# IIT-PAVIS/Acoustic-Image-Generation

Hardware: AMD Instinct MI355X
Metric: train-step images/sec (higher is better)
Workload: dtype f32

## Files before the change

acoustic-image-generation_amd/acimg/_lib.py:

```python
import ctypes as C
import os

_HERE = os.path.dirname(os.path.abspath(__file__))
LIB_PATH = os.environ.get("ACIMG_LIB") or os.path.join(_HERE, "lib", "libacimg.so")

ACT_NONE, ACT_RELU, ACT_SIGMOID = 0, 1, 2


class ConvDesc(C.Structure):

    _fields_ = [(n, C.c_int32) for n in (
        "N", "H", "W", "C", "ldx", "K", "ldy", "OH", "OW", "R", "S", "stride", "pad_t", "pad_l",
        "ldw", "act")]

    def __repr__(self):
        return "ConvDesc(" + ", ".join("%s=%d" % (n, getattr(self, n)) for n, _ in self._fields_) + ")"


class Config(C.Structure):

    _fields_ = [(n, C.c_int32) for n in (
        "splitk_cut", "splitk_target", "splitk_handoff", "wgrad_minpix", "wgrad_halo", "split3_tile_bm",
        "split3_tile_bn", "tail_split", "tail_s", "trunk_persistent", "trunk_bk", "trunk_stagger", "trunk_dma_pos",
        "trunk_ring", "trunk_ring_bm", "trunk_halo")]
# ... 33 lines not shown
    "acimg_conv2d_split3_weight_bytes": (_SZ, [_DP]),
    "acimg_conv2d_split3_prepare": (_I, [_DP, _P, _P, _P]),
    "acimg_conv2d_bf16_prepare": (_I, [_DP, _P, _P, _P]),
    "acimg_conv2d_fwd_split3_stats_rows": (_I, [_DP]),
    "acimg_conv2d_fwd_split3_tiling": (_I, [_DP, C.POINTER(C.c_int)]),
    "acimg_conv2d_fwd_split3p_stats_rows": (_I, [_DP]),
    "acimg_conv2d_fwd_split3": (_I, [_DP, _P, _P, _P, _P, _P, _P, _I, _P, _P]),
    "acimg_conv2d_fwd_bf16": (_I, [_DP, _P, _P, _P, _P, _P, _P, _I, _P, _P]),
    "acimg_conv2d_split3_dgrad_weight_bytes": (_SZ, [_DP]),
    "acimg_conv2d_split3_prepare_dgrad": (_I, [_DP, _P, _P, _P]),
    "acimg_conv2d_dgrad_split3": (_I, [_DP, _P, _I, _P, _P, _I, _P, _I, _P, _I, _P]),
    "acimg_conv2d_dgrad_bf16": (_I, [_DP, _P, _I, _P, _P, _I, _P, _I, _P, _I, _P]),
    "acimg_conv2d_split3_prepare_multi": (_I, [_I, _P, _P, _P, _P, _P]),
    "acimg_conv2d_fwd_split3p_workspace": (_SZ, [_DP]),
    "acimg_conv2d_fwd_split3p": (_I, [_DP, _P, _SZ, _P, _P, _P, _P, _SZ, _P]),
    "acimg_conv2d_fwd_split1p": (_I, [_DP, _P, _SZ, _P, _P, _P, _P, _SZ, _P]),
    "acimg_conv2d_fwd_split3p_stats": (_I, [_DP, _P, _SZ, _P, _P, _P, _SZ, _P]),
    "acimg_gram_stats_workspace": (_SZ, [_L, _I]),
    "acimg_gram_stats": (_I, [_P, _SZ, _L, _I, _P, _I, _I, _P, _P, _P, _P, _F, _F, _P, _P, _P, _SZ, _P]),
    "acimg_conv2d_fwd_split3p_tail": (_I, [_DP, _P, _SZ, _P, _P, _P, _P, _SZ, _P, _SZ, _P, _SZ, _P]),
    "acimg_conv2d_fwd_split3p_tail_proj": (_I, [_DP, _P, _SZ, _P, _P, _P, _P, _P, _P, _P, _SZ, _P, _SZ, _P]),
    "acimg_split_plane_bytes": (_SZ, [_L, _I]),
    "acimg_bn_relu_split": (_I, [_P, _P, _P, _I, _P, _SZ, _L, _I, _P]),
    "acimg_bn_add_relu_split": (_I, [_P, _P, _P, _P, _P, _P, _P, _SZ, _P, _SZ, _P, _I, _I, _I, _I, _I, _I, _I, _P]),
    "acimg_bn_relu_maxpool_split": (_I, [_P, _P, _P, _P, _SZ, _I, _I, _I, _I, _I, _I, _I, _I, _P]),
    "acimg_conv2d_dgrad": (_I, [_DP, _P, _I, _P, _P, _I, _P, _I, _P, _I, _P, _SZ, _P, _P]),
    "acimg_conv2d_dgrad_workspace": (_SZ, [_DP]),
    "acimg_conv2d_wgrad": (_I, [_DP, _P, _P, _I, _P, _P, _P, _SZ, _P]),
    "acimg_conv2d_wgrad_workspace": (_SZ, [_DP]),
    "acimg_conv2d_wgrad_split3": (_I, [_DP, _P, _P, _I, _P, _P, _P, _SZ, _P]),
# ... 140 lines not shown
```

acoustic-image-generation_amd/acimg/ops.py:

```python
import ctypes as C
import math

import torch

from . import _lib
from ._lib import ACT_NONE, ACT_RELU, ACT_SIGMOID, ConvDesc


def up4(v):
    return (int(v) + 3) & ~3


class Ptr(object):

    __slots__ = ("t", "off")

    def __init__(self, t, off=0):
        self.t = t
        self.off = int(off)

    def addr(self):
        return self.t.data_ptr() + 4 * self.off


# ... 418 lines not shown
    plan.add("conv2d_dgrad_bf16" if bf16 else "conv2d_dgrad_split3", fn, C.byref(d), gy, int(ldgy), wsplit_t, dx,
             int(lddx), residual, int(ldres), mask, int(ldmask))


def conv2d_fwd_split3p_workspace(d):
    return int(_L().acimg_conv2d_fwd_split3p_workspace(C.byref(d)))


def conv2d_fwd_split3p(plan, d, x_planes, x_lo_off, wsplit, y, stats=None, tail_ws=None, terms=3, side=False):
    nbytes = 0 if tail_ws is None else (tail_ws.numel() * tail_ws.element_size() if hasattr(tail_ws, "numel") else 0)
    fn = _L().acimg_conv2d_fwd_split3p if terms == 3 else _L().acimg_conv2d_fwd_split1p
    plan.add("conv2d_fwd_split3p" if terms == 3 else "conv2d_fwd_split1p", fn, C.byref(d), x_planes, int(x_lo_off),
             wsplit, y, stats, tail_ws, int(nbytes), side=side)


def conv2d_fwd_split3p_stats(plan, d, x_planes, x_lo_off, wsplit, stats, tail_ws=None, side=False):
    nbytes = 0 if tail_ws is None else (tail_ws.numel() * tail_ws.element_size() if hasattr(tail_ws, "numel") else 0)
    plan.add("conv2d_fwd_split3p_stats", _L().acimg_conv2d_fwd_split3p_stats, C.byref(d), x_planes, int(x_lo_off), wsplit,
             stats, tail_ws, int(nbytes), side=side)


def gram_stats_workspace(rows, Cn):
    return int(_L().acimg_gram_stats_workspace(int(rows), int(Cn)))


def gram_stats(plan, x_planes, x_lo_off, rows, Cn, w, ldw, K, gamma, beta, moving_mean, moving_var, scale, shift, ws,
               decay=0.997, eps=1e-5, side=False):
    plan.add("gram_stats", _L().acimg_gram_stats, x_planes, int(x_lo_off), int(rows), int(Cn), w, int(ldw), int(K), gamma,
             beta, moving_mean, moving_var, float(decay), float(eps), scale, shift, ws,
             int(ws.numel() * ws.element_size()), side=side)
# ... 321 lines not shown
```

acoustic-image-generation_amd/acimg/unet_acresnet.py:

```python
import os
from collections import OrderedDict

import numpy as np
import torch

from . import ops
from .ops import ACT_NONE, ACT_RELU, ACT_SIGMOID, Ptr
from .params import FusedHeads, Var, up4
from .session import get_default_session
from .vision import load_state_file

Z = 150


class Act(object):

    def __init__(self, t, N, H, W, C, ld=None, off=0):
        self.t, self.N, self.H, self.W, self.C = t, N, H, W, C
        self.ld = up4(C) if ld is None else ld
        self.off = off

    @property
    def ptr(self):
        return Ptr(self.t, self.off)
# ... 3 lines not shown
        return up4(self.C)

    @property
    def pixels(self):
        return self.N * self.H * self.W


class UNetAc(object):

    def __init__(self, input_shape=None, num_frames=12, embedding=False, num_skip=1, precision="split", side_lane=True):
        assert precision in ("split", "f32")
        self.precision = precision
        self.split_min_rows = 16384
        self.side_lane = bool(side_lane)
        self._wsplit_bufs = {}
        self.scope = 'UNetAcRes'
        self.num_frames = num_frames
        self.height = input_shape[0]
        self.width = input_shape[1]
        self.channels = input_shape[2]
        self.embedding = bool(embedding)
        self.num_skip = int(num_skip)
        assert self.num_skip in (0, 1, 2)
        self.session = None

    def _conv_specs(self):
        ns = self.num_skip
        return OrderedDict([
            ("final", (3, 3, 64, 12)),
            ("layer7/conv_2", (3, 3, 64, 64)), ("layer7/conv_1", (3, 3, 128, 64)),
# ... 132 lines not shown
        return ops.conv_desc(x.N, x.H, x.W, x.Cp if x.off == 0 and x.ld == x.Cp else x.C, K, 3, 3, stride, "SAME",
                             ldx=x.ld, ldy=(y.ld if y is not None else up4(K)), ldw=up4(K), act=act)

    def _use_split(self, d):
        return (self.precision == "split" and d.stride == 1 and d.C % 32 == 0 and d.K % 32 == 0 and
                d.N * d.OH * d.OW >= self.split_min_rows)

    def _wsplit(self, name, nbytes, kind):
        key = (name, kind)
        if key not in self._wsplit_bufs:
            self._wsplit_bufs[key] = torch.zeros(int(nbytes), dtype=torch.uint8, device=self.session.device)
        return self._wsplit_bufs[key]

    def _prepare_job(self, plan, d, name, image, mode):
        if getattr(self, "_prep_jobs", None) is None:
            (ops.conv2d_split3_prepare_dgrad if mode else ops.conv2d_split3_prepare)(plan, d, self._P(name + "/kernel"),
                                                                                      image)
            return
        self._prep_jobs.add(d, self._P(name + "/kernel"), image, mode)

    def _conv(self, plan, name, x, y, stride=1, act=ACT_RELU):
        d = self._desc(x, y.C, stride, y, act)
        self._descs[name] = (d, x, y)
        if self._use_split(d):
            ws = self._wsplit(name, ops.conv2d_split3_weight_bytes(d), "fwd")
            self._prepare_job(plan, d, name, ws, 0)
            ops.conv2d_fwd_split3(plan, d, x.ptr, ws, y.ptr, bias=self._P(name + "/bias"))
        else:
            ops.conv2d_fwd(plan, d, x.ptr, self._P(name + "/kernel"), self._P(name + "/bias"), y.ptr)

    def _record_forward(self, plan):
        N = self.N
        self._descs = {}
        h, w = self.pool1.H, self.pool1.W
        self._prep_jobs = None
        if self.precision == "split":
            self._prep_jobs = ops.PrepareJobs()
            ops.conv2d_split3_prepare_multi(plan, self._prep_jobs)
        self._conv(plan, "layer1/conv_1", self.inp, self.c11)
        self._conv(plan, "layer1/conv_2", self.c11, self.conv1)
        self._conv(plan, "layer1/pool_2", self.conv1, self.pool1, stride=3)
        self._conv(plan, "layer2/conv_1", self.pool1, self.c21)
        self._conv(plan, "layer2/conv_2", self.c21, self.conv2_0)
        ops.minmax_fwd(plan, self.conv2_0.ptr, self.conv2_0.ld, self.cat145, 148, self.mm_a, N, h * w, 133)
        ops.minmax_fwd(plan, self.feat.ptr, 12, Ptr(self.cat145, 133), 148, self.mm_b, N, h * w, 12)
        kin = h * w * 148
        self.d_heads = ops.conv_desc(N, 1, 1, kin, self.hn if not self.embedding else Z, 1, 1, 1, "VALID",
                                     ldx=kin, ldy=self.hn, ldw=self.hn)
        ops.conv2d_fwd(plan, self.d_heads, self.cat145, self._P("heads/kernel"), self._P("heads/bias"),
                       self.heads_out)
        if self.embedding:
            ops.minmax_fwd(plan, self.heads_out, self.hn, self.zbuf, 152, self.mm_z, N, 1, Z)
        else:
            ops.latent_fwd(plan, self.heads_out, self.eps, self.zbuf, 152, self.sigma, self.kl, N, Z)
        self.d_dense = ops.conv_desc(N, 1, 1, 152, 2304, 1, 1, 1, "VALID", ldx=152, ldy=2304, ldw=2304,
                                     act=ACT_RELU)
        ops.conv2d_fwd(plan, self.d_dense, self.zbuf, self._P("dense/kernel"), self._P("dense/bias"), self.dns.t)
        self._conv(plan, "conv2d", self.dns, self.net)
        self._conv(plan, "layer4/conv_1", self.l4in, self.c41)
        self._conv(plan, "layer4/conv_2", self.c41, self.conv4)
        self._conv(plan, "layer5/conv_1", self.conv4, self.c51)
        self._conv(plan, "layer5/conv_2", self.c51, self.conv5)
        self.d_up = ops.deconv_desc(N, h, w, 128, 128, 2, 2, 3, ldx=128, ldy=self.up.ld, ldw=128)
        ops.deconv_fwd(plan, self.d_up, self.conv5.ptr, self._P("upsample_1/kernel"), self._P("upsample_1/bias"),
                       self.up.ptr)
        self._conv(plan, "layer6/conv_1", self.l6in, self.c61)
        self._conv(plan, "layer6/conv_2", self.c61, self.conv6)
        self._conv(plan, "layer7/conv_1", self.conv6, self.c71)
        self._conv(plan, "layer7/conv_2", self.c71, self.conv7)
        self._conv(plan, "final", self.conv7, self.yhat, act=ACT_SIGMOID)

    def record_backward(self, plan, g_logit, g_feat, kl_weight, on_ready=None):
        on_ready = on_ready or (lambda name: None)
        N = self.N
        z = self.session.zeros
        H, W, h, w = self.height, self.width, self.pool1.H, self.pool1.W
        ns = self.num_skip

        def gbuf(a, full=False):
            return Act(z(a.N, a.H, a.W, up4(a.C)), a.N, a.H, a.W, a.C)

        def back(name, gy, dx=None, mask=None, res=None):
            d, x, y = self._descs[name]
# ... 86 lines not shown
```

acoustic-image-generation_amd/csrc/common.hpp:

```cpp
#pragma once
#include <hip/hip_runtime.h>
#include <cstdarg>
#include <cstdint>
#include <cstdio>
#include <cstring>

#include "../../include/acimg.h"

namespace acimg {

inline char* err_buf() {
    static thread_local char buf[512] = {0};
    return buf;
}
inline int fail(int code, const char* fmt, ...) {
    va_list ap;
    va_start(ap, fmt);
    vsnprintf(err_buf(), 512, fmt, ap);
    va_end(ap);
    return code;
}
inline int check_launch(const char* what) {
    hipError_t e = hipGetLastError();
    if (e != hipSuccess) return fail(ACIMG_ELAUNCH, "%s: %s", what, hipGetErrorString(e));
// ... 37 lines not shown
}

constexpr float SPLIT3_WSCALE = 1024.f;
constexpr float SPLIT3_ASCALE = 0.25f;
constexpr float SPLIT3_OUTSCALE = 1.f / 256.f;
typedef _Float16 h16x8 __attribute__((ext_vector_type(8)));
typedef _Float16 h16x4 __attribute__((ext_vector_type(4)));

__device__ __forceinline__ void split4_scaled(const float4 v, uint2& hi, uint2& lo) {
    const h16x4 h = {(_Float16)v.x, (_Float16)v.y, (_Float16)v.z, (_Float16)v.w};
    const h16x4 l = {(_Float16)(v.x - (float)h[0]), (_Float16)(v.y - (float)h[1]), (_Float16)(v.z - (float)h[2]),
                     (_Float16)(v.w - (float)h[3])};
    hi = __builtin_bit_cast(uint2, h);
    lo = __builtin_bit_cast(uint2, l);
}
__device__ __forceinline__ float4 unsplit4(const uint2 hi, const uint2 lo, float inv_scale) {
    const h16x4 h = __builtin_bit_cast(h16x4, hi), l = __builtin_bit_cast(h16x4, lo);
    return make_float4(((float)h[0] + (float)l[0]) * inv_scale, ((float)h[1] + (float)l[1]) * inv_scale,
                       ((float)h[2] + (float)l[2]) * inv_scale, ((float)h[3] + (float)l[3]) * inv_scale);
}

__device__ __forceinline__ float apply_act(float v, int act) {
    if (act == ACIMG_ACT_RELU) return fmaxf(v, 0.f);
    if (act == ACIMG_ACT_SIGMOID) return 1.f / (1.f + __expf(-v));
    return v;
}

}
```

acoustic-image-generation_amd/csrc/elementwise.hip:

```cpp
#include "common.hpp"

namespace acimg {

template <int CPB>
__global__ __launch_bounds__(1024) void bn_finalize_kernel(
    const float* stats, int rows, int C, int ld, double count, const float* gamma, const float* beta,
    float* moving_mean, float* moving_var, float decay, float eps, int training, float* scale,
    float* shift, float* save_mean, float* save_invstd) {
    constexpr int NRG = 1024 / CPB;
    constexpr int Q = 4;
    static_assert(NRG % Q == 0, "row groups per combining thread");
    __shared__ double red[2][NRG][CPB];
    __shared__ double red2[2][Q][CPB];
    const int cl = threadIdx.x % CPB, rg = threadIdx.x / CPB;
    const int c = blockIdx.x * CPB + cl;
    float g = 1.f, b = 0.f, mm = 0.f, mv = 1.f;
    if (rg == 0 && c < C) {
        if (gamma) g = gamma[c];
        if (beta) b = beta[c];
        if (moving_mean) {
            mm = moving_mean[c];
            mv = moving_var[c];
        }
    }
// ... 853 lines not shown
    float s = 0.f;
    int c = -1;
    if (start < stride) {
        c = (int)(start % C);
        for (long i = start; i < total; i += stride) {
            const float e = a[i] - b[i];
            s += e * e;
        }
    }
    if (c >= 0) atomicAdd(&acc[c], s);
    __syncthreads();
    if (threadIdx.x < C) atomicAdd(&out[threadIdx.x], acc[threadIdx.x]);
}


__device__ __forceinline__ unsigned plane_off(unsigned f, unsigned c, unsigned CQ) {
    return ((f >> 4) * CQ + (c >> 5)) * 1024u + ((f & 15u) << 6) + ((((c >> 3) ^ (0u - (f >> 2))) & 3u) << 4) + ((c & 4u) << 1);
}
struct BrickItem {
    unsigned pix, c, off;
};
__device__ __forceinline__ BrickItem brick_item(unsigned u, unsigned CQ, bool pow2, int sh) {
    const unsigned l = u & 63u, hb = u >> 6;
    const unsigned ph = pow2 ? hb >> sh : hb / CQ;
    const unsigned cq = hb - ph * CQ;
    BrickItem it;
    it.pix = ph * 8u + (l >> 3);
    it.c = cq * 32u + (l & 7u) * 4u;
    it.off = plane_off(it.pix, it.c, CQ);
    return it;
}

__global__ __launch_bounds__(256) void bn_relu_split_kernel(const float* x, const float* scale, const float* shift,
// ... 511 lines not shown
```

acoustic-image-generation_amd/csrc/igemm.hip:

```cpp
#include "wgrad_split3_kernel.hpp"
#include "igemm_split3d_kernel.hpp"
#include "igemm_split3dp_kernel.hpp"
#include "igemm_split3r_kernel.hpp"
#include "igemm_split3h_kernel.hpp"
#include "skinny_kernel.hpp"
#include <cstdlib>
#include <algorithm>
#include <type_traits>

namespace acimg {

__global__ __launch_bounds__(256) void igemm_splitk_reduce_kernel(const float* slab, int splits,
                                                                  int M, int Ngemm, int slab_ld,
                                                                  const EpiParams e) {
    const long idx = (long)blockIdx.x * 256 + threadIdx.x;
    const long total = (long)M * Ngemm;
    if (idx >= total) return;
    const int m = (int)(idx / Ngemm);
    const int n = (int)(idx - (long)m * Ngemm);
    float v = 0.f;
    for (int z = 0; z < splits; ++z) v += slab[((long)z * M + m) * slab_ld + n];
    if (n >= e.Nstore) return;
    int cn, pixoff, r, q, oh, ow;
    epi_col(e, n, cn, pixoff, r, q);
// ... 2632 lines not shown
int acimg_conv2d_split3_prepare_multi(int n, const AcimgConvDesc* const* descs, const float* const* w, void* const* out,
                                      const int* mode, void* stream) {
    if (n == 0) return ACIMG_OK;
    if (n < 0 || n > 16 || !descs || !w || !out || !mode)
        return fail(ACIMG_EINVAL, "conv2d_split3_prepare_multi: need 0..16 jobs and non-null tables");
    PrepJobs jobs{};
    jobs.n = n;
    int blocks = 0;
    for (int i = 0; i < n; ++i) {
        const AcimgConvDesc* d = descs[i];
        int rc = check_desc(d, "conv2d_split3_prepare_multi", true);
        if (rc) return rc;
        if (!w[i] || !out[i]) return fail(ACIMG_EINVAL, "conv2d_split3_prepare_multi: null pointer in job %d", i);
        PrepJob& J = jobs.j[i];
        J.w = w[i]; J.out = out[i]; J.ntaps = d->R * d->S; J.C = d->C; J.K = d->K; J.ldw = d->ldw;
        if (mode[i] < 0 || mode[i] > 2) return fail(ACIMG_EINVAL, "conv2d_split3_prepare_multi: job %d: mode is 0, 1 or 2", i);
        J.dgrad = mode[i];
        int tiles_n;
        if (J.dgrad == 1) {
            if (d->K % 32 || d->K > d->ldw)
                return fail(ACIMG_EINVAL, "conv2d_split3_prepare_multi: job %d: K must be a multiple of 32", i);
            J.Nrows = d->C;
            J.tiles_k = cdiv(d->R * d->S * d->K, 32);
            tiles_n = cdiv(d->C, 32);
        } else {
            J.Nrows = d->ldw;
            J.tiles_k = cdiv(d->R * d->S * d->C, 32);
            tiles_n = cdiv(d->ldw, 32);
        }
        J.block0 = blocks;
        blocks += J.tiles_k * tiles_n;
    }
    hipLaunchKernelGGL(split3_prepare_multi_kernel, dim3(blocks), dim3(256), 0, (hipStream_t)stream, jobs);
    return check_launch("split3_prepare_multi");
// ... 203 lines not shown

struct Split3pTail {
    int mode;
    const float* scale;
    const float* shift;
    const void* sc_planes;
    size_t sc_lo_off;
    void* out_planes;
    size_t out_lo_off;
    const float* scale2;
    const float* shift2;
};

static int fwd_presplit(const AcimgConvDesc* d, const void* x_planes, size_t x_lo_off, const void* wsplit, float* y,
                        float* stats, void* ws, size_t ws_bytes, void* stream, const int terms,
                        const Split3pTail* tail = nullptr) {
    int rc = check_desc(d, "conv2d_fwd_split3p");
    if (rc) return rc;
    if (d->C % 32) return fail(ACIMG_EINVAL, "conv2d_fwd_split3p: C=%d must be a multiple of 32", d->C);
    if (d->ldw < d->K || !aligned16(x_planes) || !aligned16(wsplit) || !aligned16(y) || (d->ldy & 3) || d->ldx != d->C ||
        (x_lo_off & 15))
        return fail(ACIMG_EINVAL, "conv2d_fwd_split3p: ldw<K, ldx != C (split-format tensors are dense) or unaligned operands");
    IgemmParams p{};
    p.A = static_cast<const float*>(x_planes); p.H = d->H; p.W = d->W; p.C = d->C; p.lda = d->ldx;
    p.OH = d->OH; p.OW = d->OW; p.R = d->R; p.S = d->S; p.stride = d->stride;
    p.pad_t = d->pad_t; p.pad_l = d->pad_l;
    p.M = d->N * d->OH * d->OW;
    p.B = static_cast<const float*>(wsplit); p.Nld = d->ldw; p.Ngemm = d->K;
    p.ntaps = d->R * d->S;
    p.kiters = p.ntaps * (d->C / 32);
    p.splits = 1;
    const long plane = (long)acimg_split_plane_bytes((long)d->N * d->H * d->W, d->C);
    const long a_bytes = (long)x_lo_off + plane;
    const long b_bytes = (long)acimg_conv2d_split3_weight_bytes(d);
    if (a_bytes >= (1L << 31) || b_bytes >= (1L << 31) || (long)x_lo_off < plane)
        return fail(ACIMG_EINVAL, "conv2d_fwd_split3p: operand >= 2 GiB or overlapping planes");
    p.a_bytes = (unsigned)a_bytes; p.b_bytes = (unsigned)b_bytes; p.a_lo_off = (unsigned)x_lo_off;
    p.b_brick = (unsigned)split3_rowmajor_bytes(d);
    EpiParams& e = p.e;
    e.Y = y; e.ldy = d->ldy; e.M = p.M; e.Nstore = d->K; e.act = d->act;
    e.stats = stats; e.stats_ld = d->ldw; e.vec = 1;
    Split3Cfg c = pick_split3(p.M, d->K);
    hipStream_t st = (hipStream_t)stream;
    p.ras_tiles_m = cdiv(p.M, c.bm);
    p.ras_tiles_n = cdiv(d->K, c.bn);
    p.ras_gn = std::min(p.ras_tiles_n, 8);
    p.ras_gm = std::max(1, 64 / p.ras_gn);
    const size_t lds_bytes = std::max((size_t)2 * 2 * (c.bm + c.bn) * 64, (size_t)c.bm * c.bn * 4) + 4 * 2 * c.bn * 4;
    const int T = p.ras_tiles_m * p.ras_tiles_n;
    const int which = (c.bm == 128 && c.bn == 128) ? 0 : (c.bm == 64 ? 1 : 2);
    const void* fn = which == 0 ? (const void*)igemm_split3d_kernel<128, 128, 2, 4, 512, 2, 2>
                   : which == 1 ? (const void*)igemm_split3d_kernel<64, 128, 1, 4, 256, 2, 2>
                                : (const void*)igemm_split3d_kernel<128, 64, 2, 2, 256, 2, 2>;
    const bool big_out = (long)p.M * d->ldy * 4 >= (1L << 31);
    if (tail) {
        if (terms != 3 || c.bm != 128 || c.bn != 128 || big_out || d->K % 128 || d->ldy != d->K || d->ldw != d->K)
// ... 25 lines not shown
        e.f_out = static_cast<char*>(tail->out_planes); e.f_out_lo = (unsigned)tail->out_lo_off;
        e.f_out_bytes = (unsigned)(tail->out_lo_off + oplane);
        if (tail->mode == 3) {
            e.f_scale2 = tail->scale2; e.f_shift2 = tail->shift2;
            e.f_sc_lo = 0; e.f_sc_bytes = (unsigned)((long)p.M * d->K * 4);
            hipLaunchKernelGGL((igemm_split3dp_kernel<32, 0, 3, 3>), dim3(nwg), dim3(512), lds_t, st, p, units, nwg);
            return check_launch("conv2d_fwd_split3p_tail_proj");
        }
        if ((tail->sc_lo_off & 15) || (long)tail->sc_lo_off < oplane || (long)tail->sc_lo_off + oplane >= (1L << 31))
            return fail(ACIMG_EINVAL, "conv2d_fwd_split3p_tail: unaligned / overlapping / >= 2 GiB shortcut planes");
        e.f_sc_lo = (unsigned)tail->sc_lo_off;
        e.f_sc_bytes = (unsigned)(tail->sc_lo_off + oplane);
        hipLaunchKernelGGL((igemm_split3dp_kernel<32, 0, 3, 2>), dim3(nwg), dim3(512), lds_t, st, p, units, nwg);
        return check_launch("conv2d_fwd_split3p_tail");
    }
    if (halo_on(d, terms)) {
        const size_t lds_h = (size_t)2 * (HALO_NB * 1024 + 64) + 2 * 2 * 128 * 64;
        const void* fh = (const void*)igemm_split3h_kernel<HALO_NB>;
        static bool attr_h = false;
        if (!attr_h) {
            (void)hipFuncSetAttribute(fh, hipFuncAttributeMaxDynamicSharedMemorySize, (int)lds_h);
            attr_h = true;
        }
        const int Ph = resident_slots(7, fh, 512, lds_h);
        TailPlan th{T, 1, 0};
        if (ws && ws_bytes >= acimg_conv2d_fwd_split3p_workspace(d)) th = pick_tail(T, Ph, p.kiters, TS_MAX_UNITS);
        p.ts_whole = th.whole; p.ts_s = th.s;
        p.ts_counters = static_cast<int*>(ws);
        p.ts_partial = ws ? reinterpret_cast<float*>(static_cast<char*>(ws) + TS_COUNTER_BYTES) : nullptr;
        hipLaunchKernelGGL((igemm_split3h_kernel<HALO_NB>), dim3(th.whole + th.rem * th.s), dim3(512), lds_h, st, p);
        return check_launch("conv2d_fwd_split3p (halo)");
    }
    if (const int rr = big_out ? 0 : ring_rows(d, terms)) {
#if defined(ACIMG_STAMP) || defined(ACIMG_ABLATE)
        p.slab = g_stamp_buf;
        p.flip = g_stamp_nostore;
#endif
        p.ras_tiles_m = cdiv(p.M, rr);
        p.ras_gm = std::max(1, 32 / p.ras_gn);
        const int Tr = p.ras_tiles_m * p.ras_tiles_n;
        const size_t lds_r = (size_t)3 * 2 * (rr + 128) * 64 + 4 * 2 * 128 * 4;
        const void* fr = rr == 256 ? (const void*)igemm_split3r_kernel<4> : (const void*)igemm_split3r_kernel<2>;
        static bool attr[2] = {false, false};
        if (!attr[rr == 256]) {
            (void)hipFuncSetAttribute(fr, hipFuncAttributeMaxDynamicSharedMemorySize, (int)lds_r);
            attr[rr == 256] = true;
        }
        const int Pr = resident_slots(rr == 256 ? 5 : 6, fr, 512, lds_r);
        TailPlan tr{Tr, 1, 0};
        if (ws && ws_bytes >= acimg_conv2d_fwd_split3p_workspace(d))
            tr = pick_tail(Tr, Pr, p.kiters, TS_MAX_UNITS * 128 / rr);
        p.ts_whole = tr.whole; p.ts_s = tr.s;
        p.ts_counters = static_cast<int*>(ws);
        p.ts_partial = ws ? reinterpret_cast<float*>(static_cast<char*>(ws) + TS_COUNTER_BYTES) : nullptr;
        const int units = tr.whole + tr.rem * tr.s;
        const int nwg = std::min(units, Pr);
        p.splits = g_cfg.trunk_stagger > 0 ? 2 : 1;
        if (rr == 256) hipLaunchKernelGGL((igemm_split3r_kernel<4>), dim3(nwg), dim3(512), lds_r, st, p, units, nwg);
        else hipLaunchKernelGGL((igemm_split3r_kernel<2>), dim3(nwg), dim3(512), lds_r, st, p, units, nwg);
        return check_launch("conv2d_fwd_split3p (ring)");
    }
    const bool persistent = !big_out && split3p_persistent(c, T);
    const size_t lds_p = (size_t)2 * 4 * 128 * 64 + 4 * 2 * 128 * 4;
    TailPlan tp{T, 1, 0};
    const int P = !persistent ? resident_slots(which, fn, which == 0 ? 512 : 256, lds_bytes)
                              : resident_slots(3, (const void*)igemm_split3dp_kernel<32, 0>, 512, lds_p);
    if (ws && ws_bytes >= acimg_conv2d_fwd_split3p_workspace(d) && which == 0)
        tp = pick_tail(T, P, p.kiters, TS_MAX_UNITS);
    p.ts_whole = tp.whole; p.ts_s = tp.s;
    p.ts_counters = static_cast<int*>(ws);
    p.ts_partial = ws ? reinterpret_cast<float*>(static_cast<char*>(ws) + TS_COUNTER_BYTES) : nullptr;
    const int n_units = tp.whole + tp.rem * tp.s;
    const dim3 grid(n_units);
#if defined(ACIMG_STAMP) || defined(ACIMG_ABLATE)
    p.slab = g_stamp_buf;
    p.flip = g_stamp_nostore;
#endif
// ... 16 lines not shown
            hipLaunchKernelGGL((igemm_split3d_kernel<128, 64, 2, 2, 256, 2, 2, 1>), grid, dim3(256), lds_bytes, st, p);
    } else if (which == 0)
        hipLaunchKernelGGL((igemm_split3d_kernel<128, 128, 2, 4, 512, 2, 2>), grid, dim3(512), lds_bytes, st, p);
    else if (which == 1)
        hipLaunchKernelGGL((igemm_split3d_kernel<64, 128, 1, 4, 256, 2, 2>), grid, dim3(256), lds_bytes, st, p);
    else
        hipLaunchKernelGGL((igemm_split3d_kernel<128, 64, 2, 2, 256, 2, 2>), grid, dim3(256), lds_bytes, st, p);
    return check_launch("conv2d_fwd_split3p");
}

int acimg_conv2d_fwd_split3p(const AcimgConvDesc* d, const void* x_planes, size_t x_lo_off, const void* wsplit,
                             float* y, float* stats, void* ws, size_t ws_bytes, void* stream) {
    return fwd_presplit(d, x_planes, x_lo_off, wsplit, y, stats, ws, ws_bytes, stream, 3);
}

int acimg_conv2d_fwd_split1p(const AcimgConvDesc* d, const void* x_planes, size_t x_lo_off, const void* wsplit,
                             float* y, float* stats, void* ws, size_t ws_bytes, void* stream) {
    return fwd_presplit(d, x_planes, x_lo_off, wsplit, y, stats, ws, ws_bytes, stream, 1);
}

int acimg_conv2d_fwd_split3p_stats(const AcimgConvDesc* d, const void* x_planes, size_t x_lo_off, const void* wsplit,
                                   float* stats, void* ws, size_t ws_bytes, void* stream) {
    if (!stats) return fail(ACIMG_EINVAL, "conv2d_fwd_split3p_stats: null statistics buffer");
    const Split3pTail t{1, nullptr, nullptr, nullptr, 0, nullptr, 0, nullptr, nullptr};
    return fwd_presplit(d, x_planes, x_lo_off, wsplit, nullptr, stats, ws, ws_bytes, stream, 3, &t);
}

int acimg_conv2d_fwd_split3p_tail(const AcimgConvDesc* d, const void* x_planes, size_t x_lo_off, const void* wsplit,
                                  const float* scale, const float* shift, const void* sc_planes, size_t sc_lo_off,
                                  void* out_planes, size_t out_lo_off, void* ws, size_t ws_bytes, void* stream) {
// ... 130 lines not shown
```

acoustic-image-generation_amd/csrc/igemm.hpp:

```cpp
#pragma once
#include "common.hpp"

namespace acimg {

struct EpiParams {
    float* Y;
    int ldy;
    int M;
    int Nstore;
    const float* bias;
    const float* res;
    int ldres;
    const float* mask;
    int ldmask;
    int act;
    int scatter;
    int Ko, Sq, sc, YH, YW, AH, AW;
    int oy0, ox0;
    float* stats;
    int stats_ld;
    int vec;
    const float* f_scale;
    const float* f_shift;
    const char* f_sc;
    char* f_out;
    unsigned f_sc_bytes, f_sc_lo, f_out_bytes, f_out_lo;
    const float* f_scale2;
    const float* f_shift2;
};

struct IgemmParams {
    const float* A;
    int H, W, C, lda;
    int OH, OW;
    int R, S, stride, pad_t, pad_l;
    int M;
    int rowrun;
    int L;
    int cps;
    int kiters;
    const float* a_scale;
    const float* a_shift;
    int a_relu;
// ... 41 lines not shown
```

acoustic-image-generation_amd/csrc/igemm_kernel.hpp:

```cpp
#pragma once
#include "igemm.hpp"

namespace acimg {

using u32x4 = __attribute__((__vector_size__(4 * sizeof(unsigned int)))) unsigned int;

__device__ __forceinline__ float4 buf_load4(__amdgpu_buffer_rsrc_t rsrc, unsigned voff) {
    return __builtin_bit_cast(float4, __builtin_amdgcn_raw_buffer_load_b128(rsrc, voff, 0, 0));
}
constexpr unsigned OOB = 0x80000000u;

__device__ __forceinline__ long epi_row_pix(const EpiParams& e, int m, int& oh, int& ow) {
    oh = 0;
    ow = 0;
    if (!e.scatter) return m;
    const int hw = e.AH * e.AW;
    const int img = m / hw;
    const int rem = m - img * hw;
    const int h = rem / e.AW;
    const int w = rem - h * e.AW;
    oh = e.sc * h + e.oy0;
    ow = e.sc * w + e.ox0;
    return ((long)img * e.YH + oh) * e.YW + ow;
}
// ... 42 lines not shown
        }
        if (e.res) {
            const float4 r = *reinterpret_cast<const float4*>(e.res + opix * e.ldres + cn);
            v.x += r.x; v.y += r.y; v.z += r.z; v.w += r.w;
        }
        if (e.act != ACIMG_ACT_NONE) {
            v.x = epi_act(v.x, e.act); v.y = epi_act(v.y, e.act);
            v.z = epi_act(v.z, e.act); v.w = epi_act(v.w, e.act);
        }
        if (e.mask) {
            const float4 k = *reinterpret_cast<const float4*>(e.mask + opix * e.ldmask + cn);
            v.x = k.x > 0.f ? v.x : 0.f; v.y = k.y > 0.f ? v.y : 0.f;
            v.z = k.z > 0.f ? v.z : 0.f; v.w = k.w > 0.f ? v.w : 0.f;
        }
        *reinterpret_cast<float4*>(e.Y + opix * e.ldy + cn) = v;
    } else {
        const float vv[4] = {v.x, v.y, v.z, v.w};
#pragma unroll
        for (int k = 0; k < 4; ++k)
            if (k < nvalid) epi_store(e, opix, cn + k, vv[k]);
    }
}

__device__ __forceinline__ float row16_sum(float v) {
    v += __builtin_bit_cast(float, __builtin_amdgcn_update_dpp(0, __builtin_bit_cast(int, v), 0xB1, 0xF, 0xF, true));
    v += __builtin_bit_cast(float, __builtin_amdgcn_update_dpp(0, __builtin_bit_cast(int, v), 0x4E, 0xF, 0xF, true));
    v += __builtin_bit_cast(float, __builtin_amdgcn_update_dpp(0, __builtin_bit_cast(int, v), 0x141, 0xF, 0xF, true));
    v += __builtin_bit_cast(float, __builtin_amdgcn_update_dpp(0, __builtin_bit_cast(int, v), 0x140, 0xF, 0xF, true));
    return v;
}
// ... 409 lines not shown
```

acoustic-image-generation_amd/csrc/igemm_split3_kernel.hpp:

```cpp
#pragma once
#include "igemm_kernel.hpp"

namespace acimg {


struct SplitF16 {
    typedef _Float16 T;
    typedef h16x8 V8;
    static constexpr float ASCALE = SPLIT3_ASCALE, WSCALE = SPLIT3_WSCALE, OUTSCALE = SPLIT3_OUTSCALE;
    static __device__ __forceinline__ f32x4 mfma(V8 a, V8 b, f32x4 c) {
        return __builtin_amdgcn_mfma_f32_16x16x32_f16(a, b, c, 0, 0, 0);
    }
};
typedef __bf16 b16x8 __attribute__((ext_vector_type(8)));
typedef __bf16 b16x4 __attribute__((ext_vector_type(4)));
struct SplitBF16 {
    typedef __bf16 T;
    typedef b16x8 V8;
    static constexpr float ASCALE = 1.f, WSCALE = 1.f, OUTSCALE = 1.f;
    static __device__ __forceinline__ f32x4 mfma(V8 a, V8 b, f32x4 c) {
        return __builtin_amdgcn_mfma_f32_16x16x32_bf16(a, b, c, 0, 0, 0);
    }
};

__device__ __forceinline__ int swz(int row) { return (0 - (row >> 2)) & 3; }

template <typename TR>
__device__ __forceinline__ void split4(float4 v, uint2& hi, uint2& lo) {
    typedef typename TR::T T;
    typedef T T4 __attribute__((ext_vector_type(4)));
    if (TR::ASCALE != 1.f) { v.x *= TR::ASCALE; v.y *= TR::ASCALE; v.z *= TR::ASCALE; v.w *= TR::ASCALE; }
    const T4 h = {(T)v.x, (T)v.y, (T)v.z, (T)v.w};
    const T4 l = {(T)(v.x - (float)h[0]), (T)(v.y - (float)h[1]), (T)(v.z - (float)h[2]), (T)(v.w - (float)h[3])};
    hi = __builtin_bit_cast(uint2, h);
    lo = __builtin_bit_cast(uint2, l);
}

template <typename TR, bool DGRAD>
__device__ __forceinline__ void split3_prepare_body(const float* w, int ntaps, int C, int K, int ldw, int Nrows,
                                                    typename TR::T* out, int bx, int by, float (*tile)[33]) {
    typedef typename TR::T T;
    const int Ktot = DGRAD ? ntaps * K : ntaps * C;
    const int k0 = bx * 32, n0 = by * 32;
    const int tx = threadIdx.x & 31, ty = threadIdx.x >> 5;
#pragma unroll
    for (int i = 0; i < 4; ++i) {
        float v = 0.f;
        if constexpr (!DGRAD) {
            const int k = k0 + ty + 8 * i, n = n0 + tx;
            if (k < Ktot && n < ldw) v = w[(long)k * ldw + n];
            tile[ty + 8 * i][tx] = v;
        } else {
            const int n = n0 + ty + 8 * i, k = k0 + tx;
            if (k < Ktot && n < C) {
                const int tp = k / K, ko = k - tp * K;
                v = w[((long)(ntaps - 1 - tp) * C + n) * ldw + ko];
            }
            tile[tx][ty + 8 * i] = v;
        }
    }
    __syncthreads();
#pragma unroll
    for (int i = 0; i < 4; ++i) {
        const int n = n0 + ty + 8 * i, k = k0 + tx;
        if (n < Nrows && k < Ktot) {
            const float v = tile[tx][ty + 8 * i] * TR::WSCALE;
            const T h = (T)v;
            out[(long)n * Ktot + k] = h;
            out[((long)Nrows + n) * Ktot + k] = (T)(v - (float)h);
        }
    }
}

template <typename TR, bool DGRAD>
__global__ __launch_bounds__(256) void split3_prepare_kernel(const float* w, int ntaps, int C, int K, int ldw,
                                                             int Nrows, typename TR::T* out) {
    __shared__ float tile[32][33];
    split3_prepare_body<TR, DGRAD>(w, ntaps, C, K, ldw, Nrows, out, blockIdx.x, blockIdx.y, tile);
}

struct PrepJob {
    const float* w;
    void* out;
    int ntaps, C, K, ldw, Nrows, dgrad, tiles_k, block0;
// ... 1 lines not shown
struct PrepJobs {
    PrepJob j[16];
    int n;
};
__global__ __launch_bounds__(256) void split3_prepare_multi_kernel(const PrepJobs jobs) {
    __shared__ float tile[32][33];
    int ji = 0;
#pragma unroll 1
    for (int i = 1; i < jobs.n; ++i)
        if ((int)blockIdx.x >= jobs.j[i].block0) ji = i;
    const PrepJob& J = jobs.j[ji];
    const int lb = blockIdx.x - J.block0;
    const int bx = lb % J.tiles_k, by = lb / J.tiles_k;
    if (J.dgrad == 1)
        split3_prepare_body<SplitBF16, true>(J.w, J.ntaps, J.C, J.K, J.ldw, J.Nrows, static_cast<__bf16*>(J.out), bx, by, tile);
    else if (J.dgrad == 2)
        split3_prepare_body<SplitBF16, false>(J.w, J.ntaps, J.C, J.K, J.ldw, J.Nrows, static_cast<__bf16*>(J.out), bx, by, tile);
    else
        split3_prepare_body<SplitF16, false>(J.w, J.ntaps, J.C, J.K, J.ldw, J.Nrows, static_cast<_Float16*>(J.out), bx, by, tile);
}

template <int BM, int BN, int WGM, int WGN, int NTHR, typename TR, int TERMS = 3>
__global__ __launch_bounds__(NTHR) void igemm_split3_kernel(const IgemmParams p) {
    static_assert(TERMS == 1 || TERMS == 3, "1 = rounded operands, 3 = split product");
    typedef typename TR::V8 V8;
    constexpr int BK = 32;
    constexpr int ROWB = BK * 2;
    constexpr int A_BYTES = BM * ROWB;
    constexpr int B_BYTES = BN * ROWB;
    constexpr int STAGE = 2 * A_BYTES + 2 * B_BYTES;
// ... 200 lines not shown
```

acoustic-image-generation_amd/csrc/igemm_split3d_kernel.hpp:

```cpp
#pragma once
#include "igemm_split3_kernel.hpp"

namespace acimg {

typedef __attribute__((address_space(3))) void* lds_ptr_t;

__device__ __forceinline__ unsigned brick_a_off(unsigned f, unsigned c32, unsigned kc) {
    return (f >> 4) * c32 + ((f & 15u) << 6) + (((kc ^ (0u - (f >> 2))) & 3u) << 4);
}
__device__ __forceinline__ unsigned brick_b_off(unsigned n, unsigned ksteps, unsigned pch) {
    return (n >> 7) * ksteps * 16384u + ((n & 127u) << 6) + (pch << 4);
}

template <int N>
__device__ __forceinline__ void wait_vmcnt() {
    static_assert(N >= 0 && N < 64, "vmcnt immediate");
    if constexpr (N == 0) asm volatile("s_waitcnt vmcnt(0)" ::: "memory");
    else if constexpr (N == 1) asm volatile("s_waitcnt vmcnt(1)" ::: "memory");
    else if constexpr (N == 2) asm volatile("s_waitcnt vmcnt(2)" ::: "memory");
    else if constexpr (N == 3) asm volatile("s_waitcnt vmcnt(3)" ::: "memory");
    else if constexpr (N == 4) asm volatile("s_waitcnt vmcnt(4)" ::: "memory");
    else if constexpr (N == 6) asm volatile("s_waitcnt vmcnt(6)" ::: "memory");
    else if constexpr (N == 8) asm volatile("s_waitcnt vmcnt(8)" ::: "memory");
    else if constexpr (N == 9) asm volatile("s_waitcnt vmcnt(9)" ::: "memory");
// ... 249 lines not shown
        for (int i = 0; i < TM; ++i)
#pragma unroll
            for (int j = 0; j < TN; ++j) acc[i][j] = f32x4{0.f, 0.f, 0.f, 0.f};
        for (int c = 0; c < p.ts_s; ++c) {
            const __amdgpu_buffer_rsrc_t rsQ =
                __builtin_amdgcn_make_buffer_rsrc(slot0 + (long)c * (BM * BN), 0, BM * BN * 4, 0x00020000);
#pragma unroll
            for (int i = 0; i < TM; ++i)
#pragma unroll
                for (int j = 0; j < TN; ++j)
                    acc[i][j] += __builtin_bit_cast(f32x4, __builtin_amdgcn_raw_buffer_load_b128(
                                                               rsQ, ((i * TN + j) * NTHR + tid) * 16, 0, 16));
        }
    }
    const EpiParams& e = p.e;
    if (e.vec && !e.bias && !e.res && !e.mask && !e.scatter && e.act == ACIMG_ACT_NONE) {
        constexpr int CH = BN / 4;
        f32x4* tile = reinterpret_cast<f32x4*>(smem);
        float* red = smem + BM * BN;
        if (e.stats) {
#pragma unroll
            for (int j = 0; j < TN; ++j) {
                f32x4 s1 = acc[0][j], s2 = acc[0][j] * acc[0][j];
#pragma unroll
                for (int i = 1; i < TM; ++i) {
                    s1 += acc[i][j];
                    s2 += acc[i][j] * acc[i][j];
                }
#pragma unroll
                for (int k = 0; k < 4; ++k) {
                    s1[k] = row16_sum(s1[k]);
// ... 62 lines not shown
```

include/acimg.h:

```cpp
#ifndef ACIMG_H_
#define ACIMG_H_

#include <stddef.h>
#include <stdint.h>

#ifdef __cplusplus
extern "C" {
#endif

#define ACIMG_VERSION 207

#define ACIMG_OK 0
#define ACIMG_EINVAL (-1)
#define ACIMG_EWORKSPACE (-2)
#define ACIMG_ELAUNCH (-3)

#define ACIMG_ACT_NONE 0
#define ACIMG_ACT_RELU 1
#define ACIMG_ACT_SIGMOID 2

int acimg_version(void);
int acimg_last_error(char* buf, size_t len);

typedef struct AcimgConvDesc {
// ... 48 lines not shown
                              int lddx, const float* residual, int ldres, const float* mask, int ldmask,
                              void* stream);

int acimg_conv2d_bf16_prepare(const AcimgConvDesc* d, const float* w, void* wsplit, void* stream);
int acimg_conv2d_fwd_bf16(const AcimgConvDesc* d, const float* x, const void* wsplit, const float* bias,
                          float* y, const float* in_scale, const float* in_shift, int in_relu, float* stats,
                          void* stream);
int acimg_conv2d_dgrad_bf16(const AcimgConvDesc* d, const float* gy, int ldgy, const void* wsplit_t, float* dx,
                            int lddx, const float* residual, int ldres, const float* mask, int ldmask,
                            void* stream);

size_t acimg_conv2d_fwd_split3p_workspace(const AcimgConvDesc* d);
int acimg_conv2d_fwd_split3p_stats_rows(const AcimgConvDesc* d);
int acimg_conv2d_fwd_split3p(const AcimgConvDesc* d, const void* x_planes, size_t x_lo_off, const void* wsplit,
                             float* y, float* stats, void* ws, size_t ws_bytes, void* stream);
int acimg_conv2d_fwd_split1p(const AcimgConvDesc* d, const void* x_planes, size_t x_lo_off, const void* wsplit,
                             float* y, float* stats, void* ws, size_t ws_bytes, void* stream);
int acimg_conv2d_fwd_split3p_stats(const AcimgConvDesc* d, const void* x_planes, size_t x_lo_off, const void* wsplit,
                                   float* stats, void* ws, size_t ws_bytes, void* stream);
int acimg_conv2d_fwd_split3p_tail(const AcimgConvDesc* d, const void* x_planes, size_t x_lo_off, const void* wsplit,
                                  const float* scale, const float* shift, const void* sc_planes, size_t sc_lo_off,
                                  void* out_planes, size_t out_lo_off, void* ws, size_t ws_bytes, void* stream);
int acimg_conv2d_fwd_split3p_tail_proj(const AcimgConvDesc* d, const void* x_planes, size_t x_lo_off, const void* wsplit,
                                       const float* scale, const float* shift, const float* sc32, const float* sc_scale,
                                       const float* sc_shift, void* out_planes, size_t out_lo_off, void* ws, size_t ws_bytes,
                                       void* stream);
size_t acimg_gram_stats_workspace(long rows, int C);
int acimg_gram_stats(const void* x_planes, size_t x_lo_off, long rows, int C, const float* w, int ldw, int K,
                     const float* gamma, const float* beta, float* moving_mean, float* moving_var, float decay, float eps,
                     float* scale, float* shift, void* ws, size_t ws_bytes, void* stream);
// ... 193 lines not shown
```

Measured before the change: 5067.

## Route decoder convs through pre-split plane path with fused bias/act and plane output

Decoder convolutions whose inputs are dense now use the pre-split plane GEMM path. Activations are split into hi/lo fp16 planes once, and the producing conv's epilogue writes both the fp32 output and the split planes for the next conv, so the next conv skips its own on-the-fly splitting. It adds a brick-layout weight prepare mode, bias, activation and plane-output support in the epilogue, and extra plane buffers. The general path disables the halo, ring and persistent kernel variants, which may cost efficiency, and the epilogue writes more bytes.

```diff
diff --git a/acoustic-image-generation_amd/acimg/_lib.py b/acoustic-image-generation_amd/acimg/_lib.py
--- a/acoustic-image-generation_amd/acimg/_lib.py
+++ b/acoustic-image-generation_amd/acimg/_lib.py
@@ -71,6 +71,7 @@
     "acimg_conv2d_split3_prepare_multi": (_I, [_I, _P, _P, _P, _P, _P]),
     "acimg_conv2d_fwd_split3p_workspace": (_SZ, [_DP]),
     "acimg_conv2d_fwd_split3p": (_I, [_DP, _P, _SZ, _P, _P, _P, _P, _SZ, _P]),
+    "acimg_conv2d_fwd_split3p_planes": (_I, [_DP, _P, _SZ, _P, _P, _P, _P, _SZ, _P, _SZ, _P]),
     "acimg_conv2d_fwd_split1p": (_I, [_DP, _P, _SZ, _P, _P, _P, _P, _SZ, _P]),
     "acimg_conv2d_fwd_split3p_stats": (_I, [_DP, _P, _SZ, _P, _P, _P, _SZ, _P]),
     "acimg_gram_stats_workspace": (_SZ, [_L, _I]),
diff --git a/acoustic-image-generation_amd/acimg/ops.py b/acoustic-image-generation_amd/acimg/ops.py
--- a/acoustic-image-generation_amd/acimg/ops.py
+++ b/acoustic-image-generation_amd/acimg/ops.py
@@ -456,6 +456,16 @@
              wsplit, y, stats, tail_ws, int(nbytes), side=side)
 
 
+def conv2d_fwd_split3p_planes(plan, d, x_planes, x_lo_off, wsplit, y, bias=None, y_planes=None, y_lo_off=0, tail_ws=None):
+    nbytes = 0 if tail_ws is None else tail_ws.numel() * tail_ws.element_size()
+    plan.add("conv2d_fwd_split3p_planes", _L().acimg_conv2d_fwd_split3p_planes, C.byref(d), x_planes, int(x_lo_off),
+             wsplit, bias, y, y_planes, int(y_lo_off), tail_ws, int(nbytes))
+
+
+def split_plane_bytes(rows, Cn):
+    return int(_L().acimg_split_plane_bytes(int(rows), int(Cn)))
+
+
 def conv2d_fwd_split3p_stats(plan, d, x_planes, x_lo_off, wsplit, stats, tail_ws=None, side=False):
     nbytes = 0 if tail_ws is None else (tail_ws.numel() * tail_ws.element_size() if hasattr(tail_ws, "numel") else 0)
     plan.add("conv2d_fwd_split3p_stats", _L().acimg_conv2d_fwd_split3p_stats, C.byref(d), x_planes, int(x_lo_off), wsplit,
diff --git a/acoustic-image-generation_amd/acimg/unet_acresnet.py b/acoustic-image-generation_amd/acimg/unet_acresnet.py
--- a/acoustic-image-generation_amd/acimg/unet_acresnet.py
+++ b/acoustic-image-generation_amd/acimg/unet_acresnet.py
@@ -41,6 +41,9 @@
         self.split_min_rows = 16384
         self.side_lane = bool(side_lane)
         self._wsplit_bufs = {}
+        self.planes = True
+        self._plane_bufs = {}
+        self._tail_ws = None
         self.scope = 'UNetAcRes'
         self.num_frames = num_frames
         self.height = input_shape[0]
@@ -203,15 +206,42 @@
 
     def _prepare_job(self, plan, d, name, image, mode):
         if getattr(self, "_prep_jobs", None) is None:
-            (ops.conv2d_split3_prepare_dgrad if mode else ops.conv2d_split3_prepare)(plan, d, self._P(name + "/kernel"),
-                                                                                      image)
+            (ops.conv2d_split3_prepare_dgrad if mode == 1 else ops.conv2d_split3_prepare)(
+                plan, d, self._P(name + "/kernel"), image)
             return
         self._prep_jobs.add(d, self._P(name + "/kernel"), image, mode)
 
-    def _conv(self, plan, name, x, y, stride=1, act=ACT_RELU):
+    def _planes(self, a):
+        if id(a) not in self._plane_bufs:
+            lo = -(-ops.split_plane_bytes(a.N * a.H * a.W, a.C) // 256) * 256
+            buf = torch.zeros(2 * lo, dtype=torch.uint8, device=self.session.device)
+            self._plane_bufs[id(a)] = (a, buf, lo)
+        return self._plane_bufs[id(a)][1:]
+
+    def _input_planes(self, plan, x):
+        buf, lo = self._planes(x)
+        if id(x) not in self._planes_fresh:
+            ops.bn_relu_split(plan, x.ptr, None, None, 0, buf, lo, x.N * x.H * x.W, x.C)
+            self._planes_fresh.add(id(x))
+        return buf, lo
+
+    def _conv(self, plan, name, x, y, stride=1, act=ACT_RELU, planes_out=False):
         d = self._desc(x, y.C, stride, y, act)
         self._descs[name] = (d, x, y)
-        if self._use_split(d):
+        if self._use_split(d) and self.planes and x.off == 0 and x.ld == x.C:
+            ws = self._wsplit(name, ops.conv2d_split3_weight_bytes(d), "fwd")
+            self._prepare_job(plan, d, name, ws, 3)
+            xp, xlo = self._input_planes(plan, x)
+            yp, ylo = None, 0
+            if planes_out and y.off == 0 and y.ld == y.C:
+                yp, ylo = self._planes(y)
+                self._planes_fresh.add(id(y))
+            if self._tail_ws is None:
+                self._tail_ws = torch.zeros(ops.conv2d_fwd_split3p_workspace(d), dtype=torch.uint8,
+                                            device=self.session.device)
+            ops.conv2d_fwd_split3p_planes(plan, d, xp, xlo, ws, y.ptr, bias=self._P(name + "/bias"), y_planes=yp,
+                                          y_lo_off=ylo, tail_ws=self._tail_ws)
+        elif self._use_split(d):
             ws = self._wsplit(name, ops.conv2d_split3_weight_bytes(d), "fwd")
             self._prepare_job(plan, d, name, ws, 0)
             ops.conv2d_fwd_split3(plan, d, x.ptr, ws, y.ptr, bias=self._P(name + "/bias"))
@@ -223,6 +253,7 @@
         self._descs = {}
         h, w = self.pool1.H, self.pool1.W
         self._prep_jobs = None
+        self._planes_fresh = set()
         if self.precision == "split":
             self._prep_jobs = ops.PrepareJobs()
             ops.conv2d_split3_prepare_multi(plan, self._prep_jobs)
@@ -253,9 +284,9 @@
         self.d_up = ops.deconv_desc(N, h, w, 128, 128, 2, 2, 3, ldx=128, ldy=self.up.ld, ldw=128)
         ops.deconv_fwd(plan, self.d_up, self.conv5.ptr, self._P("upsample_1/kernel"), self._P("upsample_1/bias"),
                        self.up.ptr)
-        self._conv(plan, "layer6/conv_1", self.l6in, self.c61)
-        self._conv(plan, "layer6/conv_2", self.c61, self.conv6)
-        self._conv(plan, "layer7/conv_1", self.conv6, self.c71)
+        self._conv(plan, "layer6/conv_1", self.l6in, self.c61, planes_out=True)
+        self._conv(plan, "layer6/conv_2", self.c61, self.conv6, planes_out=True)
+        self._conv(plan, "layer7/conv_1", self.conv6, self.c71, planes_out=True)
         self._conv(plan, "layer7/conv_2", self.c71, self.conv7)
         self._conv(plan, "final", self.conv7, self.yhat, act=ACT_SIGMOID)
 
diff --git a/acoustic-image-generation_amd/csrc/common.hpp b/acoustic-image-generation_amd/csrc/common.hpp
--- a/acoustic-image-generation_amd/csrc/common.hpp
+++ b/acoustic-image-generation_amd/csrc/common.hpp
@@ -75,6 +75,9 @@
     hi = __builtin_bit_cast(uint2, h);
     lo = __builtin_bit_cast(uint2, l);
 }
+__device__ __forceinline__ unsigned plane_off(unsigned f, unsigned c, unsigned CQ) {
+    return ((f >> 4) * CQ + (c >> 5)) * 1024u + ((f & 15u) << 6) + ((((c >> 3) ^ (0u - (f >> 2))) & 3u) << 4) + ((c & 4u) << 1);
+}
 __device__ __forceinline__ float4 unsplit4(const uint2 hi, const uint2 lo, float inv_scale) {
     const h16x4 h = __builtin_bit_cast(h16x4, hi), l = __builtin_bit_cast(h16x4, lo);
     return make_float4(((float)h[0] + (float)l[0]) * inv_scale, ((float)h[1] + (float)l[1]) * inv_scale,
diff --git a/acoustic-image-generation_amd/csrc/elementwise.hip b/acoustic-image-generation_amd/csrc/elementwise.hip
--- a/acoustic-image-generation_amd/csrc/elementwise.hip
+++ b/acoustic-image-generation_amd/csrc/elementwise.hip
@@ -891,9 +891,6 @@
 }
 
 
-__device__ __forceinline__ unsigned plane_off(unsigned f, unsigned c, unsigned CQ) {
-    return ((f >> 4) * CQ + (c >> 5)) * 1024u + ((f & 15u) << 6) + ((((c >> 3) ^ (0u - (f >> 2))) & 3u) << 4) + ((c & 4u) << 1);
-}
 struct BrickItem {
     unsigned pix, c, off;
 };
diff --git a/acoustic-image-generation_amd/csrc/igemm.hip b/acoustic-image-generation_amd/csrc/igemm.hip
--- a/acoustic-image-generation_amd/csrc/igemm.hip
+++ b/acoustic-image-generation_amd/csrc/igemm.hip
@@ -2670,10 +2670,16 @@
         if (!w[i] || !out[i]) return fail(ACIMG_EINVAL, "conv2d_split3_prepare_multi: null pointer in job %d", i);
         PrepJob& J = jobs.j[i];
         J.w = w[i]; J.out = out[i]; J.ntaps = d->R * d->S; J.C = d->C; J.K = d->K; J.ldw = d->ldw;
-        if (mode[i] < 0 || mode[i] > 2) return fail(ACIMG_EINVAL, "conv2d_split3_prepare_multi: job %d: mode is 0, 1 or 2", i);
+        if (mode[i] < 0 || mode[i] > 3) return fail(ACIMG_EINVAL, "conv2d_split3_prepare_multi: job %d: mode is 0 ... 3", i);
         J.dgrad = mode[i];
         int tiles_n;
-        if (J.dgrad == 1) {
+        if (J.dgrad == 3) {
+            if (d->C % 32) return fail(ACIMG_EINVAL, "conv2d_split3_prepare_multi: job %d: tile order needs C %% 32 == 0", i);
+            J.out = static_cast<char*>(out[i]) + split3_rowmajor_bytes(d);
+            J.Nrows = cdiv(d->ldw, 128) * 128;
+            J.tiles_k = d->R * d->S * d->C / 32;
+            tiles_n = J.Nrows / 32;
+        } else if (J.dgrad == 1) {
             if (d->K % 32 || d->K > d->ldw)
                 return fail(ACIMG_EINVAL, "conv2d_split3_prepare_multi: job %d: K must be a multiple of 32", i);
             J.Nrows = d->C;
@@ -2907,7 +2913,8 @@
 
 static int fwd_presplit(const AcimgConvDesc* d, const void* x_planes, size_t x_lo_off, const void* wsplit, float* y,
                         float* stats, void* ws, size_t ws_bytes, void* stream, const int terms,
-                        const Split3pTail* tail = nullptr) {
+                        const Split3pTail* tail = nullptr, const float* bias = nullptr, void* y_planes = nullptr,
+                        size_t y_lo_off = 0) {
     int rc = check_desc(d, "conv2d_fwd_split3p");
     if (rc) return rc;
     if (d->C % 32) return fail(ACIMG_EINVAL, "conv2d_fwd_split3p: C=%d must be a multiple of 32", d->C);
@@ -2933,6 +2940,19 @@
     EpiParams& e = p.e;
     e.Y = y; e.ldy = d->ldy; e.M = p.M; e.Nstore = d->K; e.act = d->act;
     e.stats = stats; e.stats_ld = d->ldw; e.vec = 1;
+    const bool general = bias || y_planes || d->act != ACIMG_ACT_NONE;
+    if (general) {
+        if (tail || terms != 3 || (bias && !aligned16(bias)))
+            return fail(ACIMG_EINVAL, "conv2d_fwd_split3p_planes: two-pass / fp16-operand forms or unaligned bias");
+        e.bias = bias;
+        if (y_planes) {
+            const long oplane = (long)acimg_split_plane_bytes((long)p.M, d->K);
+            if (d->K % 32 || !aligned16(y_planes) || (y_lo_off & 15) || (long)y_lo_off < oplane || oplane >= (1L << 32))
+                return fail(ACIMG_EINVAL, "conv2d_fwd_split3p_planes: K %% 32 != 0, unaligned, overlapping or >= 4 GiB output "
+                                          "planes");
+            e.p_out = static_cast<char*>(y_planes); e.p_lo = y_lo_off; e.p_cq = (unsigned)(d->K / 32);
+        }
+    }
     Split3Cfg c = pick_split3(p.M, d->K);
     hipStream_t st = (hipStream_t)stream;
     p.ras_tiles_m = cdiv(p.M, c.bm);
@@ -2988,7 +3008,7 @@
         hipLaunchKernelGGL((igemm_split3dp_kernel<32, 0, 3, 2>), dim3(nwg), dim3(512), lds_t, st, p, units, nwg);
         return check_launch("conv2d_fwd_split3p_tail");
     }
-    if (halo_on(d, terms)) {
+    if (!general && halo_on(d, terms)) {
         const size_t lds_h = (size_t)2 * (HALO_NB * 1024 + 64) + 2 * 2 * 128 * 64;
         const void* fh = (const void*)igemm_split3h_kernel<HALO_NB>;
         static bool attr_h = false;
@@ -3005,7 +3025,7 @@
         hipLaunchKernelGGL((igemm_split3h_kernel<HALO_NB>), dim3(th.whole + th.rem * th.s), dim3(512), lds_h, st, p);
         return check_launch("conv2d_fwd_split3p (halo)");
     }
-    if (const int rr = big_out ? 0 : ring_rows(d, terms)) {
+    if (const int rr = big_out || general ? 0 : ring_rows(d, terms)) {
 #if defined(ACIMG_STAMP) || defined(ACIMG_ABLATE)
         p.slab = g_stamp_buf;
         p.flip = g_stamp_nostore;
@@ -3034,7 +3054,7 @@
         else hipLaunchKernelGGL((igemm_split3r_kernel<2>), dim3(nwg), dim3(512), lds_r, st, p, units, nwg);
         return check_launch("conv2d_fwd_split3p (ring)");
     }
-    const bool persistent = !big_out && split3p_persistent(c, T);
+    const bool persistent = !big_out && !general && split3p_persistent(c, T);
     const size_t lds_p = (size_t)2 * 4 * 128 * 64 + 4 * 2 * 128 * 4;
     TailPlan tp{T, 1, 0};
     const int P = !persistent ? resident_slots(which, fn, which == 0 ? 512 : 256, lds_bytes)
@@ -3081,6 +3101,13 @@
     return fwd_presplit(d, x_planes, x_lo_off, wsplit, y, stats, ws, ws_bytes, stream, 3);
 }
 
+int acimg_conv2d_fwd_split3p_planes(const AcimgConvDesc* d, const void* x_planes, size_t x_lo_off, const void* wsplit,
+                                    const float* bias, float* y, void* y_planes, size_t y_lo_off, void* ws, size_t ws_bytes,
+                                    void* stream) {
+    return fwd_presplit(d, x_planes, x_lo_off, wsplit, y, nullptr, ws, ws_bytes, stream, 3, nullptr, bias, y_planes,
+                        y_lo_off);
+}
+
 int acimg_conv2d_fwd_split1p(const AcimgConvDesc* d, const void* x_planes, size_t x_lo_off, const void* wsplit,
                              float* y, float* stats, void* ws, size_t ws_bytes, void* stream) {
     return fwd_presplit(d, x_planes, x_lo_off, wsplit, y, stats, ws, ws_bytes, stream, 1);
diff --git a/acoustic-image-generation_amd/csrc/igemm.hpp b/acoustic-image-generation_amd/csrc/igemm.hpp
--- a/acoustic-image-generation_amd/csrc/igemm.hpp
+++ b/acoustic-image-generation_amd/csrc/igemm.hpp
@@ -27,6 +27,9 @@
     unsigned f_sc_bytes, f_sc_lo, f_out_bytes, f_out_lo;
     const float* f_scale2;
     const float* f_shift2;
+    char* p_out;
+    unsigned long p_lo;
+    unsigned p_cq;
 };
 
 struct IgemmParams {
diff --git a/acoustic-image-generation_amd/csrc/igemm_kernel.hpp b/acoustic-image-generation_amd/csrc/igemm_kernel.hpp
--- a/acoustic-image-generation_amd/csrc/igemm_kernel.hpp
+++ b/acoustic-image-generation_amd/csrc/igemm_kernel.hpp
@@ -80,6 +80,14 @@
             v.z = k.z > 0.f ? v.z : 0.f; v.w = k.w > 0.f ? v.w : 0.f;
         }
         *reinterpret_cast<float4*>(e.Y + opix * e.ldy + cn) = v;
+        if (e.p_out) {
+            uint2 hi, lo;
+            split4_scaled(make_float4(v.x * SPLIT3_ASCALE, v.y * SPLIT3_ASCALE, v.z * SPLIT3_ASCALE, v.w * SPLIT3_ASCALE),
+                          hi, lo);
+            const unsigned off = plane_off((unsigned)opix, (unsigned)cn, e.p_cq);
+            *reinterpret_cast<uint2*>(e.p_out + off) = hi;
+            *reinterpret_cast<uint2*>(e.p_out + e.p_lo + off) = lo;
+        }
     } else {
         const float vv[4] = {v.x, v.y, v.z, v.w};
 #pragma unroll
diff --git a/acoustic-image-generation_amd/csrc/igemm_split3_kernel.hpp b/acoustic-image-generation_amd/csrc/igemm_split3_kernel.hpp
--- a/acoustic-image-generation_amd/csrc/igemm_split3_kernel.hpp
+++ b/acoustic-image-generation_amd/csrc/igemm_split3_kernel.hpp
@@ -36,7 +36,7 @@
     lo = __builtin_bit_cast(uint2, l);
 }
 
-template <typename TR, bool DGRAD>
+template <typename TR, bool DGRAD, bool BRICK = false>
 __device__ __forceinline__ void split3_prepare_body(const float* w, int ntaps, int C, int K, int ldw, int Nrows,
                                                     typename TR::T* out, int bx, int by, float (*tile)[33]) {
     typedef typename TR::T T;
@@ -66,8 +66,16 @@
         if (n < Nrows && k < Ktot) {
             const float v = tile[tx][ty + 8 * i] * TR::WSCALE;
             const T h = (T)v;
-            out[(long)n * Ktot + k] = h;
-            out[((long)Nrows + n) * Ktot + k] = (T)(v - (float)h);
+            if constexpr (BRICK) {
+                const int row = n & 127;
+                const long q = (long)(n >> 7) * (Ktot >> 5) + (k >> 5);
+                const long e = ((q * 2 * 128 + row) * 4 + (((k >> 3) ^ swz(row)) & 3)) * 8 + (k & 7);
+                out[e] = h;
+                out[e + 128 * 4 * 8] = (T)(v - (float)h);
+            } else {
+                out[(long)n * Ktot + k] = h;
+                out[((long)Nrows + n) * Ktot + k] = (T)(v - (float)h);
+            }
         }
     }
 }
@@ -99,6 +107,8 @@
     const int bx = lb % J.tiles_k, by = lb / J.tiles_k;
     if (J.dgrad == 1)
         split3_prepare_body<SplitBF16, true>(J.w, J.ntaps, J.C, J.K, J.ldw, J.Nrows, static_cast<__bf16*>(J.out), bx, by, tile);
+    else if (J.dgrad == 3)
+        split3_prepare_body<SplitF16, false, true>(J.w, J.ntaps, J.C, J.K, J.ldw, J.Nrows, static_cast<_Float16*>(J.out), bx, by, tile);
     else if (J.dgrad == 2)
         split3_prepare_body<SplitBF16, false>(J.w, J.ntaps, J.C, J.K, J.ldw, J.Nrows, static_cast<__bf16*>(J.out), bx, by, tile);
     else
diff --git a/acoustic-image-generation_amd/csrc/igemm_split3d_kernel.hpp b/acoustic-image-generation_amd/csrc/igemm_split3d_kernel.hpp
--- a/acoustic-image-generation_amd/csrc/igemm_split3d_kernel.hpp
+++ b/acoustic-image-generation_amd/csrc/igemm_split3d_kernel.hpp
@@ -287,7 +287,7 @@
         }
     }
     const EpiParams& e = p.e;
-    if (e.vec && !e.bias && !e.res && !e.mask && !e.scatter && e.act == ACIMG_ACT_NONE) {
+    if (e.vec && !e.bias && !e.res && !e.mask && !e.scatter && e.act == ACIMG_ACT_NONE && !e.p_out) {
         constexpr int CH = BN / 4;
         f32x4* tile = reinterpret_cast<f32x4*>(smem);
         float* red = smem + BM * BN;
diff --git a/include/acimg.h b/include/acimg.h
--- a/include/acimg.h
+++ b/include/acimg.h
@@ -86,6 +86,9 @@
 int acimg_conv2d_fwd_split3p_stats_rows(const AcimgConvDesc* d);
 int acimg_conv2d_fwd_split3p(const AcimgConvDesc* d, const void* x_planes, size_t x_lo_off, const void* wsplit,
                              float* y, float* stats, void* ws, size_t ws_bytes, void* stream);
+int acimg_conv2d_fwd_split3p_planes(const AcimgConvDesc* d, const void* x_planes, size_t x_lo_off, const void* wsplit,
+                                    const float* bias, float* y, void* y_planes, size_t y_lo_off, void* ws, size_t ws_bytes,
+                                    void* stream);
 int acimg_conv2d_fwd_split1p(const AcimgConvDesc* d, const void* x_planes, size_t x_lo_off, const void* wsplit,
                              float* y, float* stats, void* ws, size_t ws_bytes, void* stream);
 int acimg_conv2d_fwd_split3p_stats(const AcimgConvDesc* d, const void* x_planes, size_t x_lo_off, const void* wsplit,
```

After: 5095 (median of 6 runs). Within noise of the previous version (+0.6%).
